# wangtong627/COR

Hardware: AMD Instinct MI355X
Metric: query triplets/sec (forward + similarity + top-k) (higher is better)
Workload: dtype bf16

## Files before the change

### cor_amd/_native.py

```python
from __future__ import annotations

import ctypes as C
import os

_HERE = os.path.dirname(os.path.abspath(__file__))
LIB_PATH = os.environ.get("COR_AMD_LIB") or os.path.join(_HERE, "csrc", "libcor_amd.so")

F32, BF16, F16, BF16X3 = 0, 1, 2, 3
ACT_NONE, ACT_GELU_ERF, ACT_RELU, ACT_SIGMOID, ACT_GELU_TANH = 0, 1, 2, 3, 4
EINVAL, ENOSUPPORT = -1, -2
TOPK_FORCE_LISTS, TOPK_NO_FALLBACK, TOPK_FORCE_GLOBAL_THRESHOLD, TOPK_WAVE_FINAL = 1, 2, 8, 16
TOPK_KMAX = 256
FILTER_EQ, FILTER_NE = 0, 1
MERGE_NMAX = 4096
EXPAND_SEGMAX = 16
ORDER_REVERSE = 1 << 30
KERNEL_ROWLANE, KERNEL_FEWQ, KERNEL_FLASH_MFMA, KERNEL_FLASH_PIPELINED, KERNEL_WINDOW_BLOCK = 1, 2, 3, 4, 5
import numpy as _np
Q_PRESCALE_HD64 = float(_np.float32(0.125) * _np.float32(1.4426950408889634))

_p, _i, _l, _f, _ll = C.c_void_p, C.c_int, C.c_long, C.c_float, C.c_longlong

SIGNATURES = {
    "cor_version": [],
    "cor_gemm": [_p, _l, _p, _l, _i, _p, _l, _i, _i, _i, _i, _p, _i, _p, _p, _l, _i, _i, _p],
    "cor_layernorm": [_p, _i, _p, _i, _p, _p, _i, _i, _f, _i, _p],
    "cor_attention": [_p, _l, _l, _p, _l, _l, _p, _l, _l, _i, _p, _l, _l, _i, _i, _i, _i, _i, _i, _f, _p],
    "cor_attention_f32": [_p, _l, _l, _p, _l, _l, _p, _l, _l, _p, _l, _l, _i, _i, _i, _i, _i, _i, _f, _p],
    "cor_attention_kernel_id": [_i, _i, _i, _i, _i, _i],
    "cor_sam_attention": [_p, _i, _p, _i, _p, _p, _p, _i, _i, _i, _i, _i, _f, _i, _p],
    "cor_patchify": [_p, _p, _i, _i, _i, _i, _i, _i, _i, _p],
    "cor_im2col3x3": [_p, _i, _p, _i, _i, _i, _i, _p],
    "cor_add": [_p, _i, _p, _i, _p, _i, _l, _l, _p],
    "cor_copy_rows": [_p, _l, _i, _p, _l, _i, _i, _i, _p],
    "cor_split_x3": [_p, _l, _p, _l, _l, _i, _i, _p],
    "cor_tokens_to_nchw": [_p, _i, _p, _i, _i, _i, _p],
    "cor_nchw_to_tokens": [_p, _p, _i, _i, _i, _i, _p],
    "cor_l2norm_rows": [_p, _i, _p, _i, _i, _i, _f, _p],
    "cor_embed_tokens": [_p, _p, _p, _p, _i, _i, _i, _i, _p],
    "cor_bilinear": [_p, _p, _i, _i, _i, _i, _i, _i, _p],
    "cor_conv3x3s2_small": [_p, _i, _p, _p, _p, _i, _i, _i, _i, _i, _p],
    "cor_dwconv7x7": [_p, _p, _p, _p, _i, _i, _i, _i, _i, _p],
    "cor_adapter_pool": [_p, _p, _p, _i, _i, _i, _i, _p],
    "cor_masked_pool": [_p, _i, _p, _p, _i, _i, _i, _i, _i, _p],
    "cor_region_pool": [_p, _p, _p, _p, _i, _i, _i, _i, _i, _i, _i, _p],
    "cor_fuse_gate": [_p, _p, _p, _p, _p, _i, _i, _p],
    "cor_fuse_mix": [_p, _p, _p, _i, _i, _p],
    "cor_dense_pe": [_p, _p, _i, _i, _p],
    "cor_upscale_shuffle": [_p, _i, _p, _p, _p, _f, _i, _p, _i, _i, _i, _i, _i, _p],
    "cor_upscale_hyper": [_p, _i, _p, _p, _p, _l, _p, _i, _i, _i, _i, _i, _i, _p],
    "cor_iou_select": [_p, _p, _i, _i, _i, _i, _i, _p, _p, _p],
    "cor_decoder_heads": [_p, _p, _p, _p, _p, _i, _p, _p, _i, _p],
    "cor_mask_prob_minmax": [_p, _p, _i, _i, _p],
    "cor_resize_binarize": [_p, _p, _i, _i, _i, _i, _i, _f, _p],
    "cor_resize_gray": [_p, _p, _i, _i, _i, _i, _i, _p],
    "cor_resample_rows_u8": [_p, _p, _p, _p, _i, _i, _i, _i, _i, _p],
    "cor_resample_cols_u8": [_p, _p, _p, _p, _p, _i, _i, _i, _i, _i, _p, _p, _p],
    "cor_mask_metrics": [_p, _p, _p, _i, _i, _f, _p],
    "cor_topk_workspace_bytes": [_i, _i, _i],
    "cor_similarity_topk": [_p, _p, _i, _i, _i, _i, _i, _ll, _p, _p, _p, _i, _p],
    "cor_topk_filtered_workspace_bytes": [_i, _i, _i],
    "cor_similarity_topk_filtered": [_p, _p, _i, _i, _i, _i, _i, _ll, _p, _p, _i, _p, _p, _p, _i, _p],
    "cor_topk_distinct_workspace_bytes": [_i, _i, _i],
    "cor_topk_distinct_sample_values": [_i, _i, _i],
    "cor_similarity_topk_distinct": [_p, _p, _i, _i, _i, _i, _i, _ll, _p, _p, _p, _i, _p, _p, _p, _i, _p],
    "cor_merge_topk_workspace_bytes": [_i, _i, _i, _i],
    "cor_merge_topk": [_p, _p, _p, _i, _i, _i, _i, _p, _p, _p, _p, _p],
    "cor_rescore_workspace_bytes": [_i, _i, _i],
    "cor_rescore_topk": [_p, _p, _i, _i, _i, _i, _ll, _p, _i, _i, _p, _p, _p, _p, _p],
    "cor_expand_queries": [_p, _f, _p, _p, _p, _p, _i, _p, _p, _i, _i, _i, _i, _i, _i, _p, _i, _p],
}
_RESTYPE = {"cor_topk_workspace_bytes": _l, "cor_topk_filtered_workspace_bytes": _l, "cor_topk_distinct_workspace_bytes": _l,
            "cor_merge_topk_workspace_bytes": _l, "cor_rescore_workspace_bytes": _l}

_lib = None


class NativeError(RuntimeError):
    pass


def use_probe_library():
    global LIB_PATH, _lib
    if _lib is not None:
        raise RuntimeError("use_probe_library() must be called before the library is first loaded")
    LIB_PATH = os.path.join(os.path.dirname(_HERE), "tools", "probes", "libcor_probes.so")


def load():
    global _lib
    if _lib is not None:
        return _lib
    import torch
    if not os.path.exists(LIB_PATH):
        raise ImportError(
            f"cor_amd: HIP extension not built ({LIB_PATH} missing). There is no CPU fallback. "
            "Build it with: python -c 'import __graft_entry__ as g; g.build()'  (or make -C cor_amd/csrc)")
    lib = C.CDLL(LIB_PATH)
    for name, args in SIGNATURES.items():
        fn = getattr(lib, name)
        fn.argtypes = args
        fn.restype = _RESTYPE.get(name, _i)
    _lib = lib
    return lib

# ... 10 lines not shown
```

### cor_amd/engine.py

```python
from __future__ import annotations

import math

import torch

from . import _native as nat
from . import ops
from .ops import ACT_NONE, ACT_GELU_ERF, ACT_RELU, ACT_SIGMOID, ACT_GELU_TANH, X3

F32 = torch.float32


def _round_up(x, m):
    return (x + m - 1) // m * m


class _Packer:

    def __init__(self, sd: dict, T: torch.dtype):
        dev = next(iter(sd.values())).device
        if dev.type != "cuda":
            raise RuntimeError("cor_amd: the model must live on a GPU (model.to('cuda')); there is no CPU path")
        self.sd, self.T, self.W = sd, T, {}

    def f32(self, k, t=None):
        self.W[k] = (self.sd[k] if t is None else t).detach().to(F32).contiguous()

    def mat(self, k, t=None):
        t = self.sd[k] if t is None else t
        self.W[k] = ops.split_weight_x3(t) if self.T == X3 else t.detach().to(self.T).contiguous()

    def lin(self, p):
        self.mat(p + "weight")
        self.f32(p + "bias")

    def ln(self, p):
        self.f32(p + "weight")
        self.f32(p + "bias")

    def patch_embed(self, p, dim, patch):
        kp = 3 * patch * patch
        K = _round_up(kp, 16)
        self.W[p + "patch.K"] = K
        w = self.sd[p + "patch_embed.proj.weight"].detach().reshape(dim, kp)
        if K != kp:
            w = torch.nn.functional.pad(w, (0, K - kp))
        self.mat(p + "patch_embed.proj.weight", w)
        self.f32(p + "patch_embed.proj.bias")
        self.f32(p + "pos_embed", self.sd[p + "pos_embed"].detach().reshape(-1, dim))


def pack_sam_encoder(pk: _Packer, cfg: dict, p="image_encoder."):
    sd, W, d = pk.sd, pk.W, cfg["dim"]
    pk.patch_embed(p, d, cfg["patch"])
    for i in range(cfg["depth"]):
# ... 52 lines not shown
    md = g + "mask_downscaling."
    pk.f32(md + "0.weight"); pk.f32(md + "0.bias"); pk.ln(md + "1.")
    pk.f32(md + "3.weight"); pk.f32(md + "3.bias"); pk.ln(md + "4.")
    pk.mat(md + "6.weight", sd[md + "6.weight"].detach().flatten(1)); pk.f32(md + "6.bias")


def pack_fuse(pk: _Packer, f="support_branch.cir_fuse."):
    for n in ("atten_Image", "atten_Text", "dynamic_scalar"):
        pk.lin(f"{f}{n}.0."); pk.lin(f"{f}{n}.3.")


def pack_support_head(pk: _Packer, mask_pooling: str, s="support_branch."):
    pk.ln(s + "ln_channel_first."); pk.ln(s + "ln_channel_last.")
    pk.lin(s + "dim_proj.0."); pk.lin(s + "dim_proj.3.")
    pack_fuse(pk, s + "cir_fuse.")
    if mask_pooling == "MaskAdapterPooling":
        pack_mask_adapter(pk, s + "mask_pooling.")


def pack_mask_decoder(pk: _Packer, q="mask_decoder."):
    sd = pk.sd
    tr = q + "transformer."
    attn_names = []
    for i in range(2):
        L = f"{tr}layers.{i}."
        attn_names += [L + "self_attn.", L + "cross_attn_token_to_image.", L + "cross_attn_image_to_token."]
        for n in ("norm1.", "norm2.", "norm3.", "norm4."):
            pk.ln(L + n)
        pk.lin(L + "mlp.lin1."); pk.lin(L + "mlp.lin2.")
    attn_names.append(tr + "final_attn_token_to_image.")
    for a in attn_names:
        for n in ("q_proj.", "k_proj.", "v_proj.", "out_proj."):
            pk.lin(a + n)
    pk.ln(tr + "norm_final_attn.")
    pk.f32(q + "out_tokens", torch.cat([sd[q + "iou_token.weight"], sd[q + "mask_tokens.weight"]], 0).detach().reshape(-1))
    w0 = sd[q + "output_upscaling.0.weight"].detach()
    pk.mat(q + "output_upscaling.0.weight", w0.permute(2, 3, 1, 0).reshape(4 * w0.shape[1], w0.shape[0]))
    pk.f32(q + "output_upscaling.0.bias", sd[q + "output_upscaling.0.bias"].detach().repeat(4))
    pk.ln(q + "output_upscaling.1.")
    pk.f32(q + "output_upscaling.3.weight"); pk.f32(q + "output_upscaling.3.bias")
    for i in range(4):
        for j in range(3):
            pk.lin(f"{q}output_hypernetworks_mlps.{i}.layers.{j}.")
    for j in range(3):
        pk.lin(f"{q}iou_prediction_head.layers.{j}.")
    names = [f"{q}output_hypernetworks_mlps.{i}.layers." for i in range(4)] + [f"{q}iou_prediction_head.layers."]
    last = [tuple(sd[n + "2.weight"].shape) for n in names]
    if (all(tuple(sd[n + f"{j}.weight"].shape) == (256, 256) for n in names for j in (0, 1))
            and last == [(32, 256)] * 4 + [(4, 256)]):
        pk.mat(q + "heads.w01", torch.stack([torch.stack([sd[n + "0.weight"].detach(), sd[n + "1.weight"].detach()]) for n in names]))
        pk.f32(q + "heads.b01", torch.stack([torch.stack([sd[n + "0.bias"].detach(), sd[n + "1.bias"].detach()]) for n in names]))
        pk.mat(q + "heads.w2", torch.cat([sd[n + "2.weight"].detach() for n in names], 0))
        pk.f32(q + "heads.b2", torch.cat([sd[n + "2.bias"].detach() for n in names], 0))


def pack(sd: dict, scfg: dict, gcfg: dict, mask_pooling: str, T: torch.dtype, Q=None) -> dict:
    pk = _Packer(sd, T)
    pkq = pk if Q is None or Q == T else _Packer(sd, Q)
    pack_sam_encoder(pk, scfg)
    pack_prompt_encoder(pk)
    pack_siglip(pkq, gcfg)
    pack_support_head(pkq, mask_pooling)
    pack_mask_decoder(pk)
    if pkq is not pk:
        pk.W.update(pkq.W)
    return pk.W


def _lin(W, p, a, out_dtype, act=ACT_NONE, residual=None, col_scale=None, out=None, reverse=False, x3=False):
    return ops.gemm(a, W[p + "weight"], out_dtype=out_dtype, bias=W[p + "bias"], act=act, residual=residual,
                    col_scale=col_scale, out=out, reverse=reverse, x3=x3)


def _ln(W, p, x, eps, out_dtype, act=ACT_NONE, reverse=False):
    return ops.layernorm(x, W[p + "weight"], W[p + "bias"], eps, out_dtype=out_dtype, act=act, reverse=reverse)


def _gelu(kind):
    return ACT_GELU_ERF if kind == "erf" else ACT_GELU_TANH


def sam_encoder(W, img, cfg, T, p="image_encoder."):
    B = img.shape[0]
    g, d, H = cfg["img"] // cfg["patch"], cfg["dim"], cfg["heads"]
    assert img.shape[1:] == (3, cfg["img"], cfg["img"]), f"SAM input must be [B,3,{cfg['img']},{cfg['img']}], got {tuple(img.shape)}"
    cols = ops.patchify(img, cfg["patch"], W[p + "patch.K"], T)
    x = ops.gemm(cols, W[p + "patch_embed.proj.weight"], out_dtype=F32, bias=W[p + "patch_embed.proj.bias"],
                 residual=W[p + "pos_embed"], res_row_mod=g * g)
    del cols
    for i in range(cfg["depth"]):
        b = f"{p}blocks.{i}."
        win = 0 if i in cfg["global_idx"] else cfg["window"]
        h = _ln(W, b + "norm1.", x, 1e-6, T, reverse=True)
        qkv = _lin(W, b + "attn.qkv.", h, T)
        a = ops.sam_attention(qkv, W[b + "attn.pad_row"], W[b + "attn.rel_pos_h"], W[b + "attn.rel_pos_w"], B, H, g, win,
                              q_prescale=W[b + "attn.q_prescale"], reverse=True)
        del qkv
        _lin(W, b + "attn.proj.", a, F32, residual=x, out=x)
        h = _ln(W, b + "norm2.", x, 1e-6, T, reverse=True)
        m = _lin(W, b + "mlp.lin1.", h, T, act=ACT_GELU_ERF)
        _lin(W, b + "mlp.lin2.", m, F32, residual=x, out=x)
        del h, a, m
    y = ops.gemm(ops.cast(x, T), W[p + "neck.0.weight"], out_dtype=F32)
    y = _ln(W, p + "neck.1.", y, 1e-6, T)
    y = ops.gemm(ops.im2col3x3(y, B, g, g), W[p + "neck.2.weight"], out_dtype=F32)
    return _ln(W, p + "neck.3.", y, 1e-6, F32)
# ... 73 lines not shown
        b = f"{g}cnext{i}."
        dw = ops.dwconv7x7(y, W[b + "dwconv.weight"], W[b + "dwconv.bias"], N, gh, gh)
        h = _ln(W, b + "norm.", dw, 1e-6, T)
        h = _lin(W, b + "pwconv1.", h, T, act=ACT_GELU_ERF, x3=x3)
        _lin(W, b + "pwconv2.", h, F32, residual=y, col_scale=W[b + "gamma"], out=y, x3=x3)
    h = _ln(W, g + "norm.", y, 1e-6, T)
    maps = ops.gemm(h, W[g + "final.weight"], out_dtype=F32, bias=W[g + "final.bias"], x3=x3)
    M = maps.shape[1]
    return ops.adapter_pool(maps, feat, N, P, M, D), maps


def support_head(W, vis_tokens, text_feat, mask, g, mask_pooling, T, p="support_branch."):
    D = g["dim"]
    gh = g["image"] // g["patch"]
    N = vis_tokens.shape[0] // (gh * gh)
    feat = _ln(W, p + "ln_channel_first.", vis_tokens, 1e-6, F32)
    if mask_pooling == "MaskAdapterPooling":
        pooled, _ = mask_adapter_pooling(W, feat, mask, N, gh, D, T, p + "mask_pooling.")
    else:
        m = ops.bilinear(mask, gh, gh) if tuple(mask.shape[-2:]) != (gh, gh) else mask
        pooled = ops.masked_pool(feat, m, N, gh * gh, D)
    img = _ln(W, p + "ln_channel_last.", pooled, 1e-6, F32)
    f = p + "cir_fuse."
    x3 = T == X3
    if x3:
        raw = torch.empty((N, 6 * D), dtype=torch.bfloat16, device=img.device)
        ops.split_x3(img, raw, seg=2 * D)
        ops.split_x3(text_feat, raw[:, D:], seg=2 * D)
    else:
        raw = torch.empty((N, 2 * D), dtype=T, device=img.device)
        ops.copy_rows(img, D, N, D, raw, ld_out=2 * D)
        ops.copy_rows(text_feat, D, N, D, raw[:, D:], ld_out=2 * D)

    def gate(name, x):
        h = _lin(W, f"{f}{name}.0.", x, T, act=ACT_RELU, x3=x3)
        return _lin(W, f"{f}{name}.3.", h, F32, act=ACT_SIGMOID, x3=x3)

    cat = ops.fuse_gate(img, text_feat, gate("atten_Image", raw), gate("atten_Text", raw))
    dyn = gate("dynamic_scalar", ops.cast(cat, T))
    fused = ops.fuse_mix(cat, dyn)
    h = _lin(W, p + "dim_proj.0.", ops.cast(fused, T), T, act=ACT_GELU_ERF, x3=x3)
    h = _lin(W, p + "dim_proj.3.", h, F32, act=ACT_GELU_ERF, x3=x3)
    return ops.l2norm_rows(h)


def _dec_attn(W, p, q, k, v, B, Tq, Tk, T, residual=None, out=None):
    qp, kp, vp = _lin(W, p + "q_proj.", q, T), _lin(W, p + "k_proj.", k, T), _lin(W, p + "v_proj.", v, T)
    internal = qp.shape[1]
    hd = internal // 8
    o = ops.attention(qp, kp, vp, B, 8, Tq, Tk, hd, 1.0 / math.sqrt(hd), out_dtype=T)
    return _lin(W, p + "out_proj.", o, F32, residual=residual, out=out)


def mask_decoder(W, emb_tokens, feat, T, multimask_output, all_masks=False, p="mask_decoder.", trace=None, fused_heads=True):
    B = feat.shape[0]
    Tk, Tq, C = emb_tokens.shape[0] // B, 6, 256
    g = int(math.isqrt(Tk))
    tokens = torch.empty((B * Tq, C), dtype=F32, device=feat.device)
    ops.copy_rows(W[p + "out_tokens"], 0, B, 5 * C, tokens.view(B, Tq * C), ld_out=Tq * C)
    ops.copy_rows(feat, C, B, C, tokens.view(B, Tq * C)[:, 5 * C:], ld_out=Tq * C)
    keys = ops.add(emb_tokens, W["prompt.no_mask"])
    key_pe = W["prompt.dense_pe"]
    tr = p + "transformer."
    queries = tokens
    tok_T = ops.cast(tokens, T)
    for i in range(2):
        L = f"{tr}layers.{i}."
        if i == 0:
            queries = _dec_attn(W, L + "self_attn.", tok_T, tok_T, tok_T, B, Tq, Tq, T)
        else:
            qpe = ops.add(queries, tokens, out_dtype=T)
            queries = _dec_attn(W, L + "self_attn.", qpe, qpe, ops.cast(queries, T), B, Tq, Tq, T, residual=queries)
        queries = _ln(W, L + "norm1.", queries, 1e-5, F32)
        qpe = ops.add(queries, tokens, out_dtype=T)
        kpe = ops.add(keys, key_pe, out_dtype=T)
        keys_T = ops.cast(keys, T)
        queries = _dec_attn(W, L + "cross_attn_token_to_image.", qpe, kpe, keys_T, B, Tq, Tk, T, residual=queries)
        queries = _ln(W, L + "norm2.", queries, 1e-5, F32)
        h = _lin(W, L + "mlp.lin1.", ops.cast(queries, T), T, act=ACT_RELU)
        queries = _lin(W, L + "mlp.lin2.", h, F32, residual=queries)
        queries = _ln(W, L + "norm3.", queries, 1e-5, F32)
        qpe = ops.add(queries, tokens, out_dtype=T)
        keys = _dec_attn(W, L + "cross_attn_image_to_token.", kpe, qpe, ops.cast(queries, T), B, Tk, Tq, T, residual=keys)
        keys = _ln(W, L + "norm4.", keys, 1e-5, F32)
        if trace is not None:
            trace[f"tokens_l{i}"], trace[f"keys_l{i}"] = queries, keys
    qpe = ops.add(queries, tokens, out_dtype=T)
    kpe = ops.add(keys, key_pe, out_dtype=T)
    keys_T = ops.cast(keys, T)
    queries = _dec_attn(W, tr + "final_attn_token_to_image.", qpe, kpe, keys_T, B, Tq, Tk, T, residual=queries)
    hs = _ln(W, tr + "norm_final_attn.", queries, 1e-5, T)

    if (p + "heads.w01") in W and fused_heads:
        hyper, iou = ops.decoder_heads(hs, W[p + "heads.w01"], W[p + "heads.b01"], W[p + "heads.w2"], W[p + "heads.b2"])
    else:
        hs3 = hs.view(B, Tq * C)
        hyper = torch.empty((B, 4, 32), dtype=F32, device=feat.device)
        for i in range(4):
            m = f"{p}output_hypernetworks_mlps.{i}.layers."
            a = hs3[:, (1 + i) * C:(2 + i) * C]
            a = _lin(W, m + "0.", a, T, act=ACT_RELU)
            a = _lin(W, m + "1.", a, T, act=ACT_RELU)
            _lin(W, m + "2.", a, F32, out=hyper.view(B, 128)[:, 32 * i:32 * (i + 1)])
        m = p + "iou_prediction_head.layers."
        a = _lin(W, m + "0.", hs3[:, 0:C], T, act=ACT_RELU)
        a = _lin(W, m + "1.", a, T, act=ACT_RELU)
        iou = _lin(W, m + "2.", a, F32)

    y = _lin(W, p + "output_upscaling.0.", keys_T, T)
    u1 = ops.upscale_shuffle(y, B, g, g, 64, ln_w=W[p + "output_upscaling.1.weight"], ln_b=W[p + "output_upscaling.1.bias"],
                             eps=1e-6, act=ACT_GELU_ERF)
    w3, b3 = W[p + "output_upscaling.3.weight"], W[p + "output_upscaling.3.bias"]
    k_off, ksel = (1, 3) if multimask_output else (0, 1)
    best, hyper_sel = ops.iou_select(iou, hyper, k_off, ksel)
    final = ops.upscale_hyper(u1, w3, b3, hyper_sel, B, 2 * g, 2 * g, 1)
    masks_all = ops.upscale_hyper(u1, w3, b3, hyper, B, 2 * g, 2 * g, 4) if all_masks else None
    if trace is not None:
        trace.update(hs=hs, upscaled1=u1, hyper=hyper, iou=iou, masks_all=masks_all)
    return final, iou, best, masks_all, keys


OVERLAP_BRANCHES = False
_SIDE = {}


def _side_stream(device, which=0):
    key = (device.type, device.index, which)
    if key not in _SIDE:
        _SIDE[key] = torch.cuda.Stream(device=device)
    return _SIDE[key]


def forward_support(W, gcfg, mask_pooling, T, support_image_inputs, change_text_inputs, support_mask_inputs, two_chains=True, text_stream=None):
    s_img = support_image_inputs.to(F32).contiguous()
    s_mask = support_mask_inputs.to(F32).contiguous()
    if not two_chains:
        vis = siglip_vision(W, s_img, gcfg, T)
        txt = siglip_text(W, change_text_inputs.to(s_img.device), gcfg, T)
        return support_head(W, vis, txt, s_mask, gcfg, mask_pooling, T)
    cur = torch.cuda.current_stream()
    side2 = text_stream
    if side2 is None:
        if torch.cuda.is_current_stream_capturing():
# ... 55 lines not shown
```

### cor_amd/ops.py

```python
from __future__ import annotations

import torch

from . import _native as nat
from ._native import ACT_NONE, ACT_GELU_ERF, ACT_RELU, ACT_SIGMOID, ACT_GELU_TANH, F32, BF16, F16

_DT = {torch.float32: F32, torch.bfloat16: BF16, torch.float16: F16}

X3 = "bf16x3"

GEMM_PROFILE = None


def _lib():
    return nat.load()


def _dt(t: torch.Tensor) -> int:
    return _DT[t.dtype]


def _s():
    return torch.cuda.current_stream().cuda_stream

# ... 549 lines not shown
    query_weight = float(query_weight)
    if Q is None and query_weight != 0.0:
        raise ValueError("expand_queries: Q may only be None with query_weight == 0")
    if Q is None and not segments:
        raise ValueError("expand_queries: neither queries nor segments: the width is unknown")
    C = Q.shape[-1] if Q is not None else segments[0][0].shape[-1]
    if Q is not None and (Q.dim() != 2 or Q.shape[0] != Bq or Q.dtype != torch.float32):
        raise ValueError(f"expand_queries: Q must be float32 [{Bq}, C], got {Q.dtype} {tuple(Q.shape)}")
    if C < 16 or C > 256 or C % 16 != 0:
        raise ValueError(f"expand_queries: the width must be a multiple of 16 up to 256, got {C}")
    if out_dtype not in _DT:
        raise ValueError(f"expand_queries: out_dtype must be float32 / bfloat16 / float16, got {out_dtype}")
    for r, o in segments:
        if r.dim() != 2 or r.shape[1] != C or r.dtype not in _DT or r.shape[0] >= 2 ** 31:
            raise ValueError(f"expand_queries: a segment must be float32 / bfloat16 / float16 [n < 2^31, {C}], got {r.dtype} {tuple(r.shape)}")
    spans = sorted((o, o + r.shape[0]) for r, o in segments if r.shape[0])
    for (_, hi), (lo, _) in zip(spans, spans[1:]):
        if lo < hi:
            raise ValueError("expand_queries: the segments' id ranges overlap")
    if out is not None and (out.shape != (Bq, C) or out.dtype != out_dtype or not out.is_contiguous()):
        raise ValueError(f"expand_queries: out must be a contiguous {out_dtype} [{Bq}, {C}] tensor")
    dev = _dev(Q, scores, idx, out, *[r for r, _ in segments])
    Q = Q.contiguous() if Q is not None else None
    scores, idx = scores.contiguous(), idx.contiguous()
    rows = [r.contiguous() for r, _ in segments]
    if out is None:
        out = torch.empty((Bq, C), dtype=out_dtype, device=dev)
    n = len(segments)
    c = nat.C
    seg_rows = (c.c_void_p * max(n, 1))(*[r.data_ptr() or None for r in rows])
    seg_off = (c.c_longlong * max(n, 1))(*[o for _, o in segments])
    seg_n = (c.c_int * max(n, 1))(*[r.shape[0] for r in rows])
    seg_dt = (c.c_int * max(n, 1))(*[_dt(r) for r in rows])
    if Bq:
        nat.check(_lib().cor_expand_queries(_p(Q) or None, query_weight, seg_rows, seg_off, seg_n, seg_dt, n, scores.data_ptr(), idx.data_ptr(),
                                            Bq, kin, int(m), C, int(alpha), int(bool(normalize)), out.data_ptr(), _DT[out_dtype], _s()),
                  "cor_expand_queries")
    return out


def decoder_heads(hs, w01, b01, w2, b2):
    _dev(hs, w01, b01, w2, b2)
    assert hs.is_contiguous() and hs.dim() == 2 and hs.shape[1] == 256 and hs.shape[0] % 6 == 0 and hs.dtype == w01.dtype == w2.dtype
    assert tuple(w01.shape) == (5, 2, 256, 256) and tuple(b01.shape) == (5, 2, 256) and tuple(w2.shape) == (132, 256) and tuple(b2.shape) == (132,)
    assert w01.is_contiguous() and w2.is_contiguous() and b01.is_contiguous() and b2.is_contiguous() and b01.dtype == b2.dtype == torch.float32
    B = hs.shape[0] // 6
    hyper = torch.empty((B, 4, 32), dtype=torch.float32, device=hs.device)
    iou = torch.empty((B, 4), dtype=torch.float32, device=hs.device)
    nat.check(_lib().cor_decoder_heads(hs.data_ptr(), w01.data_ptr(), b01.data_ptr(), w2.data_ptr(), b2.data_ptr(), _dt(hs), hyper.data_ptr(),
                                       iou.data_ptr(), B, _s()), "cor_decoder_heads")
    return hyper, iou


def mask_prob_minmax(logits):
    _dev(logits)
    x = logits.to(torch.float32).contiguous()
    B = x.shape[0]
    out = torch.empty_like(x)
    nat.check(_lib().cor_mask_prob_minmax(x.data_ptr(), out.data_ptr(), B, x.numel() // B, _s()), "cor_mask_prob_minmax")
    return out


def resize_binarize(prob, OH, OW, threshold=0.5):
    _dev(prob)
    assert prob.dtype == torch.float32 and prob.is_contiguous()
    B, H, W = prob.shape[0], prob.shape[-2], prob.shape[-1]
    assert prob.numel() == B * H * W
    out = torch.empty((B, OH, OW), dtype=torch.uint8, device=prob.device)
    nat.check(_lib().cor_resize_binarize(prob.data_ptr(), out.data_ptr(), B, H, W, OH, OW, float(threshold), _s()), "cor_resize_binarize")
    return out


def resize_gray(prob, OH, OW):
    _dev(prob)
    assert prob.dtype == torch.float32 and prob.is_contiguous()
    B, H, W = prob.shape[0], prob.shape[-2], prob.shape[-1]
    assert prob.numel() == B * H * W
    out = torch.empty((B, OH, OW), dtype=torch.uint8, device=prob.device)
    nat.check(_lib().cor_resize_gray(prob.data_ptr(), out.data_ptr(), B, H, W, OH, OW, _s()), "cor_resize_gray")
    return out


def mask_metrics(pred, gt, smooth=1e-5):
    _dev(pred, gt)
    assert pred.shape == gt.shape, f"Shape mismatch: pred {tuple(pred.shape)} vs gt {tuple(gt.shape)}"
    p, g = pred.to(torch.float32).contiguous(), gt.to(torch.float32).contiguous()
    B = p.shape[0]
    out = torch.empty((B, 5), dtype=torch.float32, device=p.device)
    nat.check(_lib().cor_mask_metrics(p.data_ptr(), g.data_ptr(), out.data_ptr(), B, p.numel() // B, float(smooth), _s()), "cor_mask_metrics")
    return out
```

### include/cor_amd.h

```cpp
#ifndef COR_AMD_H
#define COR_AMD_H

#ifdef __cplusplus
extern "C" {
#endif

#define COR_EINVAL (-1)
#define COR_ENOSUPPORT (-2)
#define COR_ORDER_REVERSE (1 << 30)
#define COR_TOPK_FORCE_LISTS 1
#define COR_TOPK_NO_FALLBACK 2
#define COR_TOPK_FORCE_GLOBAL_THRESHOLD 8
#define COR_TOPK_WAVE_FINAL 16
#define COR_TOPK_KMAX 256
#define COR_MERGE_NMAX 4096
#define COR_FILTER_EQ 0
#define COR_FILTER_NE 1

enum { COR_F32 = 0, COR_BF16 = 1, COR_F16 = 2 , COR_BF16X3 = 3  };
enum { COR_ACT_NONE = 0, COR_ACT_GELU_ERF = 1, COR_ACT_RELU = 2, COR_ACT_SIGMOID = 3, COR_ACT_GELU_TANH = 4 };

int cor_version(void);


// ... 24 lines not shown


int cor_patchify(const float* img, void* out, int out_dtype, int B, int C, int H, int W, int p, int Kpad, void* stream);

int cor_im2col3x3(const void* x, int dtype, void* out, int B, int H, int W, int C, void* stream);

int cor_add(const void* a, int a_dtype, const void* b, int b_dtype, void* out, int out_dtype, long n, long b_period, void* stream);

int cor_copy_rows(const void* in, long ld_in, int in_dtype, void* out, long ld_out, int out_dtype, int rows, int C, void* stream);

int cor_split_x3(const float* in, long ld_in, void* out, long ld_out, long seg, int rows, int C, void* stream);

int cor_tokens_to_nchw(const void* x, int dtype, float* out, int B, int HW, int C, void* stream);
int cor_nchw_to_tokens(const float* x, void* out, int out_dtype, int B, int HW, int C, void* stream);

int cor_l2norm_rows(const void* x, int x_dtype, void* y, int y_dtype, int rows, int C, float eps, void* stream);

int cor_embed_tokens(const long long* ids, const float* table, const float* pos, float* out, int rows, int ctx, int D, int vocab, void* stream);


int cor_bilinear(const float* x, float* out, int planes, int H, int W, int OH, int OW, int clamp01, void* stream);

int cor_conv3x3s2_small(const float* x, int x_channels_last, const float* w, const float* bias, float* out,
                        int B, int Cin, int Cout, int H, int W, void* stream);

int cor_dwconv7x7(const float* x, const float* w_t, const float* bias, void* out, int out_dtype, int B, int H, int W, int C, void* stream);

int cor_adapter_pool(const float* maps, const float* feat, float* out, int B, int P, int M, int D, void* stream);

int cor_masked_pool(const float* feat, int feat_nchw, const float* mask, float* out, int B, int P, int D,
                    int clamp01, int l2norm, void* stream);

int cor_region_pool(const float* tokens, const float* masks, const int* region_offsets, void* out, int out_dtype, int B, int R,
                    int P, int D, int clamp01, int l2norm, void* stream);

int cor_fuse_gate(const float* img, const float* txt, const float* aI, const float* aT, float* cat, int N, int D, void* stream);
int cor_fuse_mix(const float* cat, const float* dyn, float* out, int N, int D, void* stream);


int cor_dense_pe(const float* gauss, float* out, int size, int F, void* stream);

int cor_upscale_shuffle(const void* y, int y_dtype, const float* bias, const float* ln_w, const float* ln_b, float eps,
                        int act, void* out, int out_dtype, int B, int H, int W, int Cout, void* stream);

int cor_upscale_hyper(const void* x, int dtype, const float* w, const float* bias, const float* hyper, long hyper_bs,
                      float* masks, int B, int H, int W, int Cin, int Cout, int Kmask, void* stream);

int cor_iou_select(const float* iou, const float* hyper, int B, int Kall, int k_off, int Ksel, int C, long long* best,
                   float* hyper_sel, void* stream);

int cor_decoder_heads(const void* hs, const void* w01, const float* b01, const void* w2, const float* b2, int dtype, float* hyper,
                      float* iou, int B, void* stream);


int cor_mask_prob_minmax(const float* logits, float* out, int B, int HW, void* stream);

int cor_resize_binarize(const float* prob, unsigned char* out, int B, int H, int W, int OH, int OW, float threshold, void* stream);

int cor_resize_gray(const float* prob, unsigned char* out, int B, int H, int W, int OH, int OW, void* stream);

int cor_mask_metrics(const float* pred, const float* gt, float* out, int B, int HW, float smooth, void* stream);


int cor_resample_rows_u8(const unsigned char* in, unsigned char* out, const int* bounds, const int* kk, int ksize, int H, int W, int C,
                         int OW, void* stream);

int cor_resample_cols_u8(const unsigned char* in, float* out_f32, unsigned char* out_u8, const int* bounds, const int* kk, int ksize, int H,
                         int W, int C, int OH, const float* mean, const float* stdv, void* stream);


long cor_topk_workspace_bytes(int Bq, int Ng, int k);
int cor_similarity_topk(const float* Q, const void* G, int g_dtype, int Bq, int Ng, int C, int k, long long g_offset,
                        float* out_scores, long long* out_idx, void* workspace, int flags, void* stream);

long cor_topk_filtered_workspace_bytes(int Bq, int Ng, int k);
int cor_similarity_topk_filtered(const float* Q, const void* G, int g_dtype, int Bq, int Ng, int C, int k, long long g_offset,
                                 const int* row_labels, const int* query_labels, int filter_mode, float* out_scores, long long* out_idx,
                                 void* workspace, int flags, void* stream);

long cor_topk_distinct_workspace_bytes(int Bq, int Ng, int k);
int cor_topk_distinct_sample_values(int Bq, int Ng, int k);
int cor_similarity_topk_distinct(const float* Q, const void* G, int g_dtype, int Bq, int Ng, int C, int k, long long g_offset,
                                 const int* row_groups, const int* row_labels, const int* query_labels, int filter_mode, float* out_scores,
                                 long long* out_idx, void* workspace, int flags, void* stream);

long cor_merge_topk_workspace_bytes(int P, int Bq, int kin, int k);
int cor_merge_topk(const float* scores, const long long* idx, const int* groups, int P, int Bq, int kin, int k, float* out_scores,
                   long long* out_idx, int* out_groups, void* workspace, void* stream);

long cor_rescore_workspace_bytes(int Bq, int kin, int k);
int cor_rescore_topk(const float* Q, const void* G, int g_dtype, int Bq, int Ng, int C, long long g_offset, const long long* cand, int kin,
                     int k, float* out_scores, long long* out_idx, int* out_pos, void* workspace, void* stream);

#define COR_EXPAND_SEGMAX 16
int cor_expand_queries(const float* Q, float query_weight, const void* const* seg_rows, const long long* seg_offset, const int* seg_n,
                       const int* seg_dtype, int nseg, const float* scores, const long long* idx, int Bq, int kin, int m, int C, int alpha,
                       int normalize, void* out, int out_dtype, void* stream);

#ifdef __cplusplus
}
#endif
#endif
```

Baseline: 784.5.

## Fuse decoder image-side attention, LayerNorm and K/V/Q projections into one kernel

Adds a HIP kernel that handles the whole image-token side of each two-way transformer layer for one 64-row tile. It computes image-to-token attention, out_proj, the residual and LayerNorm, the positional-encoding add, and the next layer's k/v/q projections with bf16 MFMA, keeping intermediates in LDS. The engine routes the bf16 mask decoder through this path by default, which replaces several separate add, cast, GEMM, attention and LayerNorm launches along with their global-memory round trips. In exchange it is limited to specific shapes (width 256, internal 128, Tq up to 8) and uses a large LDS tile, which may cap occupancy.

```diff
diff --git a/cor_amd/_native.py b/cor_amd/_native.py
--- a/cor_amd/_native.py
+++ b/cor_amd/_native.py
@@ -9,6 +9,7 @@
 F32, BF16, F16, BF16X3 = 0, 1, 2, 3
 ACT_NONE, ACT_GELU_ERF, ACT_RELU, ACT_SIGMOID, ACT_GELU_TANH = 0, 1, 2, 3, 4
 EINVAL, ENOSUPPORT = -1, -2
+IMAGE_PASS_ENTRY, IMAGE_PASS_UPDATE = 0, 1
 TOPK_FORCE_LISTS, TOPK_NO_FALLBACK, TOPK_FORCE_GLOBAL_THRESHOLD, TOPK_WAVE_FINAL = 1, 2, 8, 16
 TOPK_KMAX = 256
 FILTER_EQ, FILTER_NE = 0, 1
@@ -51,6 +52,8 @@
     "cor_upscale_hyper": [_p, _i, _p, _p, _p, _l, _p, _i, _i, _i, _i, _i, _i, _p],
     "cor_iou_select": [_p, _p, _i, _i, _i, _i, _i, _p, _p, _p],
     "cor_decoder_heads": [_p, _p, _p, _p, _p, _i, _p, _p, _i, _p],
+    "cor_decoder_image_pass": [_i, _p, _p, _p, _p, _p, _p, _p, _p, _p, _f, _p, _p, _i, _p, _p, _p, _p, _p, _p, _p, _p, _p, _p, _i, _i, _i, _i,
+                               _i, _i, _i, _i, _p],
     "cor_mask_prob_minmax": [_p, _p, _i, _i, _p],
     "cor_resize_binarize": [_p, _p, _i, _i, _i, _i, _i, _f, _p],
     "cor_resize_gray": [_p, _p, _i, _i, _i, _i, _i, _p],
diff --git a/cor_amd/csrc/decoder_image.hip b/cor_amd/csrc/decoder_image.hip
--- /dev/null
+++ b/cor_amd/csrc/decoder_image.hip
@@ -0,0 +1,338 @@
+#include "common.h"
+
+namespace {
+
+constexpr int BM = 64;
+constexpr int ROWB = 1040;
+constexpr int C = 256, CI = 128;
+constexpr int HD = 16;
+constexpr int TQMAX = 8;
+
+struct ImgArgs {
+  const float* keys_in; const float* no_mask;
+  const bf16_t* q; const bf16_t* tok_k; const bf16_t* tok_v;
+  const uint4* w_out; const float* b_out; const float* ln_w; const float* ln_b; float eps;
+  float* keys_out; const float* pe; int pe_rows;
+  const uint4* w_k; const uint4* w_v; const uint4* w_q;
+  const float* b_k; const float* b_v; const float* b_q;
+  bf16_t* k_out; bf16_t* v_out; bf16_t* q_out; bf16_t* keys_t_out;
+  long M; int Tk, Tq, rev; float scale;
+};
+
+__device__ __forceinline__ f32x16 mfma_bf16(const uint4& a, const uint4& b, f32x16 acc) {
+  return __builtin_amdgcn_mfma_f32_32x32x16_bf16(__builtin_bit_cast(bf16x8, a), __builtin_bit_cast(bf16x8, b), acc, 0, 0, 0);
+}
+__device__ __forceinline__ long lmin(long x, long y) { return x < y ? x : y; }
+__device__ __forceinline__ uint2 pack4(f32x4 v) {
+  uint2 u;
+  u.x = (uint32_t)f2bf(v[0]) | ((uint32_t)f2bf(v[1]) << 16);
+  u.y = (uint32_t)f2bf(v[2]) | ((uint32_t)f2bf(v[3]) << 16);
+  return u;
+}
+template <int CTRL> __device__ __forceinline__ float dpp_add(float v) {
+  return v + __builtin_bit_cast(float, __builtin_amdgcn_update_dpp(0, __builtin_bit_cast(int, v), CTRL, 0xf, 0xf, true));
+}
+template <int N> __device__ __forceinline__ void wave_sum_n(float (&s)[N], char* scratch, int lane) {
+  static_assert(N % 4 == 0, "16-byte LDS accesses");
+#pragma unroll
+  for (int o = 32; o >= 16; o >>= 1) {
+#pragma unroll
+    for (int i = 0; i < N; i += 4) *(f32x4*)(scratch + (i / 4) * 1024 + lane * 16) = f32x4{s[i], s[i + 1], s[i + 2], s[i + 3]};
+    __builtin_amdgcn_fence(__ATOMIC_RELEASE, "wavefront");
+    __builtin_amdgcn_wave_barrier();
+    __builtin_amdgcn_fence(__ATOMIC_ACQUIRE, "wavefront");
+#pragma unroll
+    for (int i = 0; i < N; i += 4) {
+      const f32x4 t = *(const f32x4*)(scratch + (i / 4) * 1024 + (lane ^ o) * 16);
+      s[i] += t[0]; s[i + 1] += t[1]; s[i + 2] += t[2]; s[i + 3] += t[3];
+    }
+    __builtin_amdgcn_fence(__ATOMIC_RELEASE, "wavefront");
+    __builtin_amdgcn_wave_barrier();
+    __builtin_amdgcn_fence(__ATOMIC_ACQUIRE, "wavefront");
+  }
+#pragma unroll
+  for (int i = 0; i < N; ++i) {
+    float v = s[i];
+    v = dpp_add<0x128>(v);
+    v = dpp_add<0x124>(v);
+    v = dpp_add<0x4E>(v);
+    v = dpp_add<0xB1>(v);
+    s[i] = v;
+  }
+}
+__device__ __forceinline__ float dot16(const float (&q)[HD], const bf16_t* __restrict__ p) {
+  float a0 = 0.f, a1 = 0.f;
+#pragma unroll
+  for (int i = 0; i < HD / 4; ++i) {
+    const f32x4 kv = ld4<bf16_t>(p + 4 * i);
+    a0 = fmaf(q[4 * i + 0], kv[0], a0); a1 = fmaf(q[4 * i + 1], kv[1], a1);
+    a0 = fmaf(q[4 * i + 2], kv[2], a0); a1 = fmaf(q[4 * i + 3], kv[3], a1);
+  }
+  return a0 + a1;
+}
+
+template <bool UPDATE, bool HAS_Q>
+__global__ void __launch_bounds__(256, 2) decoder_image_pass(const ImgArgs a) {
+  extern __shared__ __attribute__((aligned(16))) char smem[];
+  const int tid = threadIdx.x, lane = tid & 63, wave = tid >> 6;
+  const int r = lane & 31, h = lane >> 5;
+  const long tile = a.rev ? (long)gridDim.x - 1 - blockIdx.x : (long)blockIdx.x;
+  const long m0 = tile * BM;
+  auto frag = [&](int rt, int off, int ks) { return *(const uint4*)(smem + (rt * 32 + r) * ROWB + off + (ks * 16 + 8 * h) * 2); };
+
+  f32x4 pre[BM / 4];
+#pragma unroll
+  for (int i = 0; i < BM / 4; ++i) pre[i] = *(const f32x4*)(a.keys_in + lmin(m0 + wave * (BM / 4) + i, a.M - 1) * C + 4 * lane);
+
+  if constexpr (UPDATE) {
+    {
+      const int wv = __builtin_amdgcn_readfirstlane(wave);
+      const long gm = lmin(m0 + lane, a.M - 1);
+      const unsigned tk = (unsigned)a.Tk;
+      const int bmine = (int)((unsigned)gm / tk);
+      const int b0 = (int)((unsigned)m0 / tk), b1 = (int)((unsigned)lmin(m0 + BM - 1, a.M - 1) / tk);
+      float q[2][HD];
+#pragma unroll
+      for (int hh = 0; hh < 2; ++hh)
+#pragma unroll
+        for (int i = 0; i < HD / 4; ++i) {
+          const f32x4 v4 = ld4<bf16_t>(a.q + gm * CI + (2 * wv + hh) * HD + 4 * i);
+          q[hh][4 * i] = v4[0]; q[hh][4 * i + 1] = v4[1]; q[hh][4 * i + 2] = v4[2]; q[hh][4 * i + 3] = v4[3];
+        }
+      for (int b = b0; b <= b1; ++b) {
+#pragma unroll
+        for (int hh = 0; hh < 2; ++hh) {
+          const int hc = (2 * wv + hh) * HD;
+          const bf16_t* kb = a.tok_k + (long)b * a.Tq * CI + hc;
+          const bf16_t* vb = a.tok_v + (long)b * a.Tq * CI + hc;
+          float o[HD];
+#pragma unroll
+          for (int d = 0; d < HD; ++d) o[d] = 0.f;
+          float s[TQMAX];
+          float mx = -INFINITY;
+#pragma unroll
+          for (int jj = 0; jj < TQMAX; ++jj) {
+            s[jj] = -INFINITY;
+            if (jj < a.Tq) s[jj] = dot16(q[hh], kb + jj * CI) * a.scale;
+            mx = fmaxf(mx, s[jj]);
+          }
+          float l = 0.f;
+#pragma unroll
+          for (int jj = 0; jj < TQMAX; ++jj) {
+            if (jj < a.Tq) {
+              const float p = __expf(s[jj] - mx);
+              l += p;
+              const bf16_t* vp = vb + jj * CI;
+#pragma unroll
+              for (int i = 0; i < HD / 4; ++i) {
+                const f32x4 vv = ld4<bf16_t>(vp + 4 * i);
+                o[4 * i] = fmaf(p, vv[0], o[4 * i]); o[4 * i + 1] = fmaf(p, vv[1], o[4 * i + 1]);
+                o[4 * i + 2] = fmaf(p, vv[2], o[4 * i + 2]); o[4 * i + 3] = fmaf(p, vv[3], o[4 * i + 3]);
+              }
+            }
+          }
+          const float inv = 1.0f / l;
+          if (b == bmine) {
+#pragma unroll
+            for (int i = 0; i < HD / 8; ++i) {
+              const uint2 lo = pack4(f32x4{o[8 * i] * inv, o[8 * i + 1] * inv, o[8 * i + 2] * inv, o[8 * i + 3] * inv});
+              const uint2 hi = pack4(f32x4{o[8 * i + 4] * inv, o[8 * i + 5] * inv, o[8 * i + 6] * inv, o[8 * i + 7] * inv});
+              *(uint4*)(smem + lane * ROWB + (hc + 8 * i) * 2) = make_uint4(lo.x, lo.y, hi.x, hi.y);
+            }
+          }
+        }
+      }
+    }
+    __syncthreads();
+    f32x16 acc[2][2];
+#pragma unroll
+    for (int f = 0; f < 2; ++f)
+#pragma unroll
+      for (int rt = 0; rt < 2; ++rt)
+#pragma unroll
+        for (int e = 0; e < 16; ++e) acc[f][rt][e] = 0.f;
+#pragma unroll
+    for (int ks = 0; ks < CI / 16; ++ks) {
+      uint4 wf[2], bf[2];
+#pragma unroll
+      for (int f = 0; f < 2; ++f) wf[f] = a.w_out[((2 * wave + f) * (CI / 16) + ks) * 64 + lane];
+#pragma unroll
+      for (int rt = 0; rt < 2; ++rt) bf[rt] = frag(rt, 0, ks);
+#pragma unroll
+      for (int f = 0; f < 2; ++f)
+#pragma unroll
+        for (int rt = 0; rt < 2; ++rt) acc[f][rt] = mfma_bf16(wf[f], bf[rt], acc[f][rt]);
+    }
+    __syncthreads();
+#pragma unroll
+    for (int f = 0; f < 2; ++f)
+#pragma unroll
+      for (int g = 0; g < 4; ++g) {
+        const int feat = (2 * wave + f) * 32 + 8 * g + 4 * h;
+        const f32x4 bv = *(const f32x4*)(a.b_out + feat);
+#pragma unroll
+        for (int rt = 0; rt < 2; ++rt) {
+          const f32x4 v = f32x4{acc[f][rt][4 * g], acc[f][rt][4 * g + 1], acc[f][rt][4 * g + 2], acc[f][rt][4 * g + 3]} + bv;
+          *(f32x4*)(smem + (rt * 32 + r) * ROWB + feat * 4) = v;
+        }
+      }
+    __syncthreads();
+  }
+
+  {
+    f32x4 wv = {0.f, 0.f, 0.f, 0.f}, bv = wv, nm = wv;
+    if constexpr (UPDATE) { wv = *(const f32x4*)(a.ln_w + 4 * lane); bv = *(const f32x4*)(a.ln_b + 4 * lane); }
+    else nm = *(const f32x4*)(a.no_mask + 4 * lane);
+    const unsigned row0 = (unsigned)__builtin_amdgcn_readfirstlane(wave) * (BM / 4);
+    const unsigned pe0 = ((unsigned)m0 + row0) % (unsigned)a.pe_rows;
+    constexpr int NR = BM / 4;
+    if constexpr (UPDATE) {
+      float s[NR], qq[NR];
+      char* scratch = smem + row0 * ROWB;
+#pragma unroll
+      for (int i = 0; i < NR; ++i) {
+        pre[i] = *(const f32x4*)(smem + (row0 + i) * ROWB + lane * 16) + pre[i];
+        s[i] = pre[i][0] + pre[i][1] + pre[i][2] + pre[i][3];
+      }
+      wave_sum_n(s, scratch, lane);
+#pragma unroll
+      for (int i = 0; i < NR; ++i) {
+        s[i] = s[i] / C;
+        qq[i] = 0.f;
+#pragma unroll
+        for (int e = 0; e < 4; ++e) { const float d = pre[i][e] - s[i]; qq[i] = fmaf(d, d, qq[i]); }
+      }
+      wave_sum_n(qq, scratch, lane);
+#pragma unroll
+      for (int i = 0; i < NR; ++i) {
+        const float rstd = 1.0f / sqrtf(qq[i] / C + a.eps);
+#pragma unroll
+        for (int e = 0; e < 4; ++e) pre[i][e] = fmaf((pre[i][e] - s[i]) * rstd, wv[e], bv[e]);
+      }
+    } else {
+#pragma unroll
+      for (int i = 0; i < NR; ++i) pre[i] = pre[i] + nm;
+    }
+#pragma unroll
+    for (int i = 0; i < NR; ++i) {
+      const long gm = m0 + row0 + i;
+      char* lrow = smem + (row0 + i) * ROWB;
+      const f32x4 pe = *(const f32x4*)(a.pe + (size_t)((pe0 + i) % (unsigned)a.pe_rows) * C + 4 * lane);
+      const f32x4 o = pre[i];
+      if (gm < a.M) *(f32x4*)(a.keys_out + gm * C + 4 * lane) = o;
+      const uint2 kt = pack4(o);
+      *(uint2*)(lrow + lane * 8) = pack4(o + pe);
+      *(uint2*)(lrow + 512 + lane * 8) = kt;
+      if (a.keys_t_out && gm < a.M) *(uint2*)(a.keys_t_out + gm * C + 4 * lane) = kt;
+    }
+  }
+  __syncthreads();
+
+  constexpr int NO = HAS_Q ? 3 : 2;
+  f32x16 acc[NO][2];
+#pragma unroll
+  for (int p = 0; p < NO; ++p)
+#pragma unroll
+    for (int rt = 0; rt < 2; ++rt)
+#pragma unroll
+      for (int e = 0; e < 16; ++e) acc[p][rt][e] = 0.f;
+#pragma unroll
+  for (int ks = 0; ks < C / 16; ++ks) {
+    const int wi = (wave * (C / 16) + ks) * 64 + lane;
+    uint4 wf[NO], bk[2], bt[2];
+    wf[0] = a.w_k[wi]; wf[1] = a.w_v[wi];
+    if constexpr (HAS_Q) wf[2] = a.w_q[wi];
+#pragma unroll
+    for (int rt = 0; rt < 2; ++rt) { bk[rt] = frag(rt, 0, ks); bt[rt] = frag(rt, 512, ks); }
+#pragma unroll
+    for (int rt = 0; rt < 2; ++rt) {
+      acc[0][rt] = mfma_bf16(wf[0], bk[rt], acc[0][rt]);
+      acc[1][rt] = mfma_bf16(wf[1], bt[rt], acc[1][rt]);
+      if constexpr (HAS_Q) acc[2][rt] = mfma_bf16(wf[2], bk[rt], acc[2][rt]);
+    }
+  }
+  __syncthreads();
+#pragma unroll
+  for (int p = 0; p < NO; ++p) {
+    const float* bias = p == 0 ? a.b_k : p == 1 ? a.b_v : a.b_q;
+#pragma unroll
+    for (int g = 0; g < 4; ++g) {
+      const int feat = wave * 32 + 8 * g + 4 * h;
+      const f32x4 bv = *(const f32x4*)(bias + feat);
+#pragma unroll
+      for (int rt = 0; rt < 2; ++rt) {
+        const f32x4 v = f32x4{acc[p][rt][4 * g], acc[p][rt][4 * g + 1], acc[p][rt][4 * g + 2], acc[p][rt][4 * g + 3]} + bv;
+        *(uint2*)(smem + (rt * 32 + r) * ROWB + p * (CI * 2) + feat * 2) = pack4(v);
+      }
+    }
+  }
+  __syncthreads();
+#pragma unroll
+  for (int p = 0; p < NO; ++p) {
+    bf16_t* out = p == 0 ? a.k_out : p == 1 ? a.v_out : a.q_out;
+#pragma unroll
+    for (int c = tid; c < BM * 16; c += 256) {
+      const int row = c >> 4, ch = c & 15;
+      const long gm = m0 + row;
+      if (gm < a.M) *(uint4*)(out + gm * CI + ch * 8) = *(const uint4*)(smem + row * ROWB + p * (CI * 2) + ch * 16);
+    }
+  }
+}
+
+DevOnce g_once[4];
+
+inline bool aligned16(const void* p) { return ((uintptr_t)p & 15) == 0; }
+
+}
+
+extern "C" int cor_decoder_image_pass(int mode, const float* keys_in, const float* no_mask, const void* q, const void* tok_k,
+                                      const void* tok_v, const void* w_out, const float* b_out, const float* ln_w, const float* ln_b,
+                                      float ln_eps, float* keys_out, const float* pe, int pe_rows, const void* w_k, const float* b_k,
+                                      const void* w_v, const float* b_v, const void* w_q, const float* b_q, void* k_out, void* v_out,
+                                      void* q_out, void* keys_t_out, int dtype, int B, int Tk, int Tq, int width, int internal, int heads,
+                                      int cfg, void* stream) {
+  if (mode != COR_IMAGE_PASS_ENTRY && mode != COR_IMAGE_PASS_UPDATE) return COR_EINVAL;
+  if (cfg & ~COR_ORDER_REVERSE) return COR_EINVAL;
+  if (B < 1 || Tk < 1 || pe_rows < 1) return COR_EINVAL;
+  if (!keys_in || !keys_out || !pe || !w_k || !b_k || !w_v || !b_v || !k_out || !v_out) return COR_EINVAL;
+  if ((w_q != nullptr) != (q_out != nullptr) || (w_q != nullptr) != (b_q != nullptr)) return COR_EINVAL;
+  const bool upd = mode == COR_IMAGE_PASS_UPDATE;
+  if (upd) {
+    if (!q || !tok_k || !tok_v || !w_out || !b_out || !ln_w || !ln_b) return COR_EINVAL;
+    if (!(ln_eps > 0.f) || Tq < 1) return COR_EINVAL;
+  } else if (!no_mask) {
+    return COR_EINVAL;
+  }
+  const void* ptrs[] = {keys_in, no_mask, q, tok_k, tok_v, w_out, b_out, ln_w, ln_b, keys_out, pe, w_k, b_k, w_v, b_v, w_q, b_q,
+                        k_out, v_out, q_out, keys_t_out};
+  for (const void* p : ptrs)
+    if (!aligned16(p)) return COR_EINVAL;
+  if (dtype != COR_BF16 || width != C || internal != CI || heads != CI / HD) return COR_ENOSUPPORT;
+  if (upd && Tq > TQMAX) return COR_ENOSUPPORT;
+  const long M = (long)B * Tk;
+  if (M > (1L << 31) - BM) return COR_ENOSUPPORT;
+
+  ImgArgs a;
+  a.keys_in = keys_in; a.no_mask = no_mask;
+  a.q = (const bf16_t*)q; a.tok_k = (const bf16_t*)tok_k; a.tok_v = (const bf16_t*)tok_v;
+  a.w_out = (const uint4*)w_out; a.b_out = b_out; a.ln_w = ln_w; a.ln_b = ln_b; a.eps = ln_eps;
+  a.keys_out = keys_out; a.pe = pe; a.pe_rows = pe_rows;
+  a.w_k = (const uint4*)w_k; a.w_v = (const uint4*)w_v; a.w_q = (const uint4*)w_q;
+  a.b_k = b_k; a.b_v = b_v; a.b_q = b_q;
+  a.k_out = (bf16_t*)k_out; a.v_out = (bf16_t*)v_out; a.q_out = (bf16_t*)q_out; a.keys_t_out = (bf16_t*)keys_t_out;
+  a.M = M; a.Tk = Tk; a.Tq = Tq; a.rev = (cfg & COR_ORDER_REVERSE) ? 1 : 0;
+  a.scale = 1.0f / sqrtf((float)HD);
+  const int lds = BM * ROWB;
+  const dim3 grid(cdiv(M, BM)), block(256);
+  hipStream_t s = (hipStream_t)stream;
+#define COR_LAUNCH(U_, Q_, I_)                                                                          \
+  do {                                                                                                  \
+    cor_max_dyn_lds((const void*)decoder_image_pass<U_, Q_>, lds, g_once[I_]);                          \
+    hipLaunchKernelGGL((decoder_image_pass<U_, Q_>), grid, block, lds, s, a);                           \
+  } while (0)
+  if (upd) { if (w_q) COR_LAUNCH(true, true, 0); else COR_LAUNCH(true, false, 1); }
+  else     { if (w_q) COR_LAUNCH(false, true, 2); else COR_LAUNCH(false, false, 3); }
+#undef COR_LAUNCH
+  COR_CHECK_LAUNCH();
+  return 0;
+}
diff --git a/cor_amd/engine.py b/cor_amd/engine.py
--- a/cor_amd/engine.py
+++ b/cor_amd/engine.py
@@ -1,6 +1,7 @@
 from __future__ import annotations
 
 import math
+import os
 
 import torch
 
@@ -159,6 +160,14 @@
         pk.f32(q + "heads.b01", torch.stack([torch.stack([sd[n + "0.bias"].detach(), sd[n + "1.bias"].detach()]) for n in names]))
         pk.mat(q + "heads.w2", torch.cat([sd[n + "2.weight"].detach() for n in names], 0))
         pk.f32(q + "heads.b2", torch.cat([sd[n + "2.bias"].detach() for n in names], 0))
+    t2i = [f"{tr}layers.{i}.cross_attn_token_to_image." for i in range(2)] + [tr + "final_attn_token_to_image."]
+    i2t = [f"{tr}layers.{i}.cross_attn_image_to_token." for i in range(2)]
+    frag = [a + n for a in t2i for n in ("k_proj.", "v_proj.")] + [a + "q_proj." for a in i2t]
+    if (pk.T == torch.bfloat16 and all(tuple(sd[n + "weight"].shape) == (128, 256) for n in frag)
+            and all(tuple(sd[a + "out_proj.weight"].shape) == (256, 128) for a in i2t)):
+        for n in frag + [a + "out_proj." for a in i2t]:
+            pk.W[n + "frag"] = ops.pack_mfma_weight(sd[n + "weight"])
+        pk.W[q + "image_pass"] = True
 
 
 def pack(sd: dict, scfg: dict, gcfg: dict, mask_pooling: str, T: torch.dtype, Q=None) -> dict:
@@ -338,6 +347,22 @@
     return _lin(W, p + "out_proj.", o, F32, residual=residual, out=out)
 
 
+DECODER_IMAGE_PASS = os.environ.get("COR_DECODER_IMAGE_PASS", "1") != "0"
+
+
+def _image_stage(W, t2i, i2t, keys_in, B, **kw):
+    wq, bq = (W[i2t + "q_proj.frag"], W[i2t + "q_proj.bias"]) if i2t else (None, None)
+    return ops.decoder_image_pass(keys_in, W["prompt.dense_pe"], B, W[t2i + "k_proj.frag"], W[t2i + "k_proj.bias"],
+                                  W[t2i + "v_proj.frag"], W[t2i + "v_proj.bias"], wq, bq, **kw)
+
+
+def _dec_attn_kv(W, p, q, kp, vp, B, Tq, Tk, T, residual):
+    qp = _lin(W, p + "q_proj.", q, T)
+    hd = qp.shape[1] // 8
+    o = ops.attention(qp, kp, vp, B, 8, Tq, Tk, hd, 1.0 / math.sqrt(hd), out_dtype=T)
+    return _lin(W, p + "out_proj.", o, F32, residual=residual)
+
+
 def mask_decoder(W, emb_tokens, feat, T, multimask_output, all_masks=False, p="mask_decoder.", trace=None, fused_heads=True):
     B = feat.shape[0]
     Tk, Tq, C = emb_tokens.shape[0] // B, 6, 256
@@ -345,9 +370,14 @@
     tokens = torch.empty((B * Tq, C), dtype=F32, device=feat.device)
     ops.copy_rows(W[p + "out_tokens"], 0, B, 5 * C, tokens.view(B, Tq * C), ld_out=Tq * C)
     ops.copy_rows(feat, C, B, C, tokens.view(B, Tq * C)[:, 5 * C:], ld_out=Tq * C)
-    keys = ops.add(emb_tokens, W["prompt.no_mask"])
+    tr = p + "transformer."
+    fused = DECODER_IMAGE_PASS and T == torch.bfloat16 and W.get(p + "image_pass", False) and Tq <= 8
+    if fused:
+        keys, k_img, v_img, q_img, _ = _image_stage(W, tr + "layers.0.cross_attn_token_to_image.", tr + "layers.0.cross_attn_image_to_token.",
+                                                    emb_tokens, B, no_mask=W["prompt.no_mask"])
+    else:
+        keys = ops.add(emb_tokens, W["prompt.no_mask"])
     key_pe = W["prompt.dense_pe"]
-    tr = p + "transformer."
     queries = tokens
     tok_T = ops.cast(tokens, T)
     for i in range(2):
@@ -359,22 +389,40 @@
             queries = _dec_attn(W, L + "self_attn.", qpe, qpe, ops.cast(queries, T), B, Tq, Tq, T, residual=queries)
         queries = _ln(W, L + "norm1.", queries, 1e-5, F32)
         qpe = ops.add(queries, tokens, out_dtype=T)
-        kpe = ops.add(keys, key_pe, out_dtype=T)
-        keys_T = ops.cast(keys, T)
-        queries = _dec_attn(W, L + "cross_attn_token_to_image.", qpe, kpe, keys_T, B, Tq, Tk, T, residual=queries)
+        if fused:
+            queries = _dec_attn_kv(W, L + "cross_attn_token_to_image.", qpe, k_img, v_img, B, Tq, Tk, T, queries)
+        else:
+            kpe = ops.add(keys, key_pe, out_dtype=T)
+            keys_T = ops.cast(keys, T)
+            queries = _dec_attn(W, L + "cross_attn_token_to_image.", qpe, kpe, keys_T, B, Tq, Tk, T, residual=queries)
         queries = _ln(W, L + "norm2.", queries, 1e-5, F32)
         h = _lin(W, L + "mlp.lin1.", ops.cast(queries, T), T, act=ACT_RELU)
         queries = _lin(W, L + "mlp.lin2.", h, F32, residual=queries)
         queries = _ln(W, L + "norm3.", queries, 1e-5, F32)
         qpe = ops.add(queries, tokens, out_dtype=T)
-        keys = _dec_attn(W, L + "cross_attn_image_to_token.", kpe, qpe, ops.cast(queries, T), B, Tk, Tq, T, residual=keys)
-        keys = _ln(W, L + "norm4.", keys, 1e-5, F32)
+        if fused:
+            a = L + "cross_attn_image_to_token."
+            upd = (q_img, _lin(W, a + "k_proj.", qpe, T), _lin(W, a + "v_proj.", ops.cast(queries, T), T), W[a + "out_proj.frag"],
+                   W[a + "out_proj.bias"], W[L + "norm4.weight"], W[L + "norm4.bias"], 1e-5)
+            if i == 0:
+                nxt = f"{tr}layers.1."
+                keys, k_img, v_img, q_img, _ = _image_stage(W, nxt + "cross_attn_token_to_image.", nxt + "cross_attn_image_to_token.",
+                                                            keys, B, update=upd, Tq=Tq)
+            else:
+                keys, k_img, v_img, _, keys_T = _image_stage(W, tr + "final_attn_token_to_image.", None, keys, B, update=upd, Tq=Tq,
+                                                             keys_T=True)
+        else:
+            keys = _dec_attn(W, L + "cross_attn_image_to_token.", kpe, qpe, ops.cast(queries, T), B, Tk, Tq, T, residual=keys)
+            keys = _ln(W, L + "norm4.", keys, 1e-5, F32)
         if trace is not None:
             trace[f"tokens_l{i}"], trace[f"keys_l{i}"] = queries, keys
     qpe = ops.add(queries, tokens, out_dtype=T)
-    kpe = ops.add(keys, key_pe, out_dtype=T)
-    keys_T = ops.cast(keys, T)
-    queries = _dec_attn(W, tr + "final_attn_token_to_image.", qpe, kpe, keys_T, B, Tq, Tk, T, residual=queries)
+    if fused:
+        queries = _dec_attn_kv(W, tr + "final_attn_token_to_image.", qpe, k_img, v_img, B, Tq, Tk, T, queries)
+    else:
+        kpe = ops.add(keys, key_pe, out_dtype=T)
+        keys_T = ops.cast(keys, T)
+        queries = _dec_attn(W, tr + "final_attn_token_to_image.", qpe, kpe, keys_T, B, Tq, Tk, T, residual=queries)
     hs = _ln(W, tr + "norm_final_attn.", queries, 1e-5, T)
 
     if (p + "heads.w01") in W and fused_heads:
diff --git a/cor_amd/ops.py b/cor_amd/ops.py
--- a/cor_amd/ops.py
+++ b/cor_amd/ops.py
@@ -625,6 +625,46 @@
     return hyper, iou
 
 
+def pack_mfma_weight(w):
+    N, K = w.shape
+    assert N % 32 == 0 and K % 16 == 0, (N, K)
+    return w.detach().to(torch.bfloat16).reshape(N // 32, 32, K // 16, 2, 8).permute(0, 2, 3, 1, 4).contiguous()
+
+
+def decoder_image_pass(keys_in, pe, B, w_k, b_k, w_v, b_v, w_q=None, b_q=None, no_mask=None, update=None, Tq=0, keys_T=False,
+                       reverse=False, width=256, internal=128, heads=8):
+    assert (no_mask is None) != (update is None)
+    upd = update if update is not None else (None,) * 7 + (0.0,)
+    q, tok_k, tok_v, w_out, b_out, ln_w, ln_b, eps = upd
+    _dev(keys_in, pe, w_k, b_k, w_v, b_v, w_q, b_q, no_mask, q, tok_k, tok_v, w_out, b_out, ln_w, ln_b)
+    M = keys_in.shape[0]
+    assert keys_in.dim() == 2 and keys_in.is_contiguous() and keys_in.dtype == torch.float32 and keys_in.shape[1] == width and M % B == 0
+    assert pe.dim() == 2 and pe.is_contiguous() and pe.dtype == torch.float32 and pe.shape[1] == width
+    for w, b, n, k in ((w_k, b_k, internal, width), (w_v, b_v, internal, width), (w_q, b_q, internal, width), (w_out, b_out, width, internal)):
+        if w is None:
+            assert b is None
+            continue
+        assert w.dtype == torch.bfloat16 and w.is_contiguous() and tuple(w.shape) == (n // 32, k // 16, 2, 32, 8), (w.shape, n, k)
+        _f32vec(b, n, "bias")
+    if update is not None:
+        for t, rows in ((q, M), (tok_k, B * Tq), (tok_v, B * Tq)):
+            assert t.dtype == torch.bfloat16 and t.is_contiguous() and tuple(t.shape) == (rows, internal), (t.shape, rows)
+        _f32vec(ln_w, width, "ln_w"); _f32vec(ln_b, width, "ln_b")
+    else:
+        assert no_mask.dtype == torch.float32 and no_mask.is_contiguous() and no_mask.numel() == width
+    dev = keys_in.device
+    keys = torch.empty((M, width), dtype=torch.float32, device=dev)
+    k_out, v_out = (torch.empty((M, internal), dtype=torch.bfloat16, device=dev) for _ in range(2))
+    q_out = torch.empty((M, internal), dtype=torch.bfloat16, device=dev) if w_q is not None else None
+    kt = torch.empty((M, width), dtype=torch.bfloat16, device=dev) if keys_T else None
+    nat.check(_lib().cor_decoder_image_pass(
+        nat.IMAGE_PASS_UPDATE if update is not None else nat.IMAGE_PASS_ENTRY, keys_in.data_ptr(), _p(no_mask), _p(q), _p(tok_k), _p(tok_v),
+        _p(w_out), _p(b_out), _p(ln_w), _p(ln_b), float(eps), keys.data_ptr(), pe.data_ptr(), pe.shape[0], w_k.data_ptr(), b_k.data_ptr(),
+        w_v.data_ptr(), b_v.data_ptr(), _p(w_q), _p(b_q), k_out.data_ptr(), v_out.data_ptr(), _p(q_out), _p(kt), nat.BF16, B, M // B, int(Tq),
+        width, internal, heads, nat.ORDER_REVERSE if reverse else 0, _s()), "cor_decoder_image_pass")
+    return keys, k_out, v_out, q_out, kt
+
+
 def mask_prob_minmax(logits):
     _dev(logits)
     x = logits.to(torch.float32).contiguous()
diff --git a/include/cor_amd.h b/include/cor_amd.h
--- a/include/cor_amd.h
+++ b/include/cor_amd.h
@@ -100,6 +100,13 @@
 int cor_decoder_heads(const void* hs, const void* w01, const float* b01, const void* w2, const float* b2, int dtype, float* hyper,
                       float* iou, int B, void* stream);
 
+enum { COR_IMAGE_PASS_ENTRY = 0, COR_IMAGE_PASS_UPDATE = 1 };
+int cor_decoder_image_pass(int mode, const float* keys_in, const float* no_mask, const void* q, const void* tok_k, const void* tok_v,
+                           const void* w_out, const float* b_out, const float* ln_w, const float* ln_b, float ln_eps, float* keys_out,
+                           const float* pe, int pe_rows, const void* w_k, const float* b_k, const void* w_v, const float* b_v,
+                           const void* w_q, const float* b_q, void* k_out, void* v_out, void* q_out, void* keys_t_out, int dtype,
+                           int B, int Tk, int Tq, int width, int internal, int heads, int cfg, void* stream);
+
 
 int cor_mask_prob_minmax(const float* logits, float* out, int B, int HW, void* stream);
 
```

After: 790.8, median of 6. No clear change (+0.8%).
